# kurhula/pyABC

Hardware: AMD Instinct MI355X
Metric: accepted particles/sec/generation (higher is better)
Workload: dtype f32 (f16x3-limb MFMA, f32-grade)

## Files before the change

### pyabc_amd/csrc/abc_mvn_x3.hip

```cpp
#include "abc_common.h"

namespace abc {
namespace {

typedef _Float16 half8 __attribute__((ext_vector_type(8)));
typedef float f32x16 __attribute__((ext_vector_type(16)));

constexpr double LOG2E = 1.4426950408889634074;
constexpr double SQRT_LOG2E = 1.2011224087864498;
constexpr double LN2 = 0.69314718055994530942;
constexpr int MAX_R = 25;
constexpr int E_MIN = 3, E_MAX = 8;
constexpr float O_MIN = -64.f;
constexpr size_t HDR = 256;
constexpr int X3_PAD = 8;
constexpr int TR = 32;

struct Header { double maxsq; int E; int ok; };

__host__ __device__ constexpr int x3_g0(int r) { return (r + 7 + 7) / 8; }
__host__ __device__ constexpr int x3_k0pad(int r) { return 8 * x3_g0(r); }
__host__ __device__ constexpr int x3_kb(int r) { return (x3_k0pad(r) + 5 * r + 4 + 15) / 16; }
__host__ __device__ constexpr int x3_kb0(int r) { return (x3_g0(r) + 1) / 2; }
static_assert(x3_kb(10) == 5, "K = 80 at r = 10");

struct Limbs3 { double a1, a2, a3; };
struct Limbs5 { double c[5]; };

__device__ __forceinline__ Limbs3 split_coord(double v, int E) {
  Limbs3 L;
  const double G = ldexp(1.0, E - 11);
  L.a1 = rint(v / G);
  double r = v - L.a1 * G;
  L.a2 = rint(ldexp(r / G, 11));
  r -= ldexp(L.a2 * G, -11);
  L.a3 = rint(ldexp(r / G, 22));
  return L;
}

__device__ __forceinline__ int scalar_exp(int l, int E) { return 2 * E - 22 + 22 - 11 * l; }

__device__ __forceinline__ Limbs5 split_scalar(double c, int E) {
  Limbs5 L;
  double r = c;
  for (int l = 0; l < 5; ++l) {
    const int e = scalar_exp(l, E);
    L.c[l] = rint(ldexp(r, -e));
    r -= ldexp(L.c[l], e);
  }
  return L;
}

__device__ __forceinline__ float opv(double limb, int e) { return (float)ldexp(limb, e); }

template <int SIDE>
__device__ __forceinline__ float slot_value(int k, int r, int K0pad, int E,
                                            const Limbs3* L, const Limbs5& S) {
  if (k < K0pad) {
    const int e0 = 2 * (E - 11);
    if (k < r) {
      const int x = e0 >> 1;
      return opv(L[k].a1, SIDE == 0 ? x : e0 - x);
    }
    const int q = k - r;
    if (q < 6) {
      const int l = q % 3;
      const int e = scalar_exp(l, E);
      const int x = e > 4 ? 4 : e;
      const bool limb_side = (q < 3) == (SIDE == 0);
      return limb_side ? opv(S.c[l], x) : opv(1.0, e - x);
    }
    if (q == 6) return SIDE == 0 ? 1.f : 0.f;
    return 0.f;
  }
  const int q = k - K0pad;
  if (q < 5 * r) {
    const int cls = q / r, dim = q % r;
    const int pa[5] = {1, 2, 1, 2, 3}, pb[5] = {2, 1, 3, 2, 1};
    const int p = SIDE == 0 ? pa[cls] : pb[cls];
    const int etot = 2 * (E - 11) - 11 * (pa[cls] + pb[cls] - 2);
    const int x = etot >> 1;
    const double limb = p == 1 ? L[dim].a1 : (p == 2 ? L[dim].a2 : L[dim].a3);
    return opv(limb, SIDE == 0 ? x : etot - x);
  }
  const int e4 = q - 5 * r;
  if (e4 < 4) {
    const int l = 3 + (e4 & 1);
    const int e = scalar_exp(l, E);
    const int x = e < -24 ? -24 : e;
    const bool limb_side = (e4 < 2) == (SIDE == 0);
    return limb_side ? opv(S.c[l], x) : opv(1.0, e - x);
  }
  return 0.f;
}

template <int RR = MAX_R>
__device__ __forceinline__ double whiten(const double* __restrict__ P, int64_t row,
                                         int d, const double* __restrict__ mu,
                                         const double* __restrict__ U, int r,
                                         double* v) {
  double acc[RR];
#pragma unroll
  for (int k = 0; k < RR; ++k) acc[k] = 0.0;
  for (int q = 0; q < d; ++q) {
    const double xq = P[row * d + q] - mu[q];
#pragma unroll
    for (int k = 0; k < RR; ++k)
      if (k < r) acc[k] += xq * U[q * r + k];
  }
  double h = 0.0;
#pragma unroll
  for (int k = 0; k < RR; ++k) {
    if (k < r) {
      const double a = acc[k] * SQRT_LOG2E;
      v[k] = a;
      h += a * a;
    }
  }
  return 0.5 * h;
}

constexpr int POP_RANGE_BLOCKS = 1024;
__global__ __launch_bounds__(256) void pop_range_kernel(
    const double* __restrict__ X, const double* __restrict__ w, int64_t N,
    int d, const double* __restrict__ mu, const double* __restrict__ U, int r,
    Header* __restrict__ hdr) {
  __shared__ double wm[4];
  double h = 0.0;
  for (int64_t row = (int64_t)blockIdx.x * blockDim.x + threadIdx.x; row < N;
       row += (int64_t)gridDim.x * blockDim.x) {
    if (w[row] > 0.0) {
      double v[MAX_R];
      h = fmax(h, whiten(X, row, d, mu, U, r, v));
    }
  }
  h = wave_max(h);
  if ((threadIdx.x & 63) == 0) wm[threadIdx.x >> 6] = h;
  __syncthreads();
  if (threadIdx.x == 0) {
    h = fmax(fmax(wm[0], wm[1]), fmax(wm[2], wm[3]));
    if (h > 0.0)
      atomicMax((unsigned long long*)&hdr->maxsq,
                (unsigned long long)__double_as_longlong(h));
  }
}

__global__ void x3_setup_kernel(Header* __restrict__ hdr, int r,
                                double* __restrict__ range) {
  const double ymax = sqrt(2.0 * hdr->maxsq);
  int E = (int)ceil(log2(1.25 * ymax + 2.0 * sqrt((double)r) + 4.0));
  if (E < E_MIN) E = E_MIN;
  hdr->E = E;
  hdr->ok = E <= E_MAX ? 1 : 0;
  if (range) { range[0] = ymax; range[1] = (double)E; }
}

template <int SIDE, int R>
__global__ __launch_bounds__(128) void pack_x3_kernel(
    const double* __restrict__ P, const double* __restrict__ w, int64_t n,
    int d, const double* __restrict__ mu, const double* __restrict__ U, int r_rt,
    double log_w_shift, int K0pad_rt, int KB_rt, const Header* __restrict__ hdr,
    _Float16* __restrict__ img, int64_t ntiles, int32_t* __restrict__ flags,
    double* __restrict__ Y, double* __restrict__ lw, int64_t Np,
    const int64_t* __restrict__ hint, float* __restrict__ cand_o, int koff,
    const double* __restrict__ shift_dev, const unsigned int* __restrict__ count_dev) {
  if (count_dev) { const int64_t c = (int64_t)*count_dev; n = c < n ? c : n; }
  constexpr int RR = R > 0 ? R : MAX_R;
  const int r = R > 0 ? R : r_rt;
  const int K0pad = R > 0 ? x3_k0pad(R) : K0pad_rt;
  const int KB = R > 0 ? x3_kb(R) : KB_rt;
  constexpr int NG = R > 0 ? x3_kb(R) * 2 : 0;
  const int64_t row = (int64_t)blockIdx.x * blockDim.x + threadIdx.x;
  if (row >= ntiles * TR) return;
  if (count_dev && (row / TR) * TR >= n) return;
  const int E = hdr->E;
  const bool ok = hdr->ok != 0;
  const double L2 = ldexp(1.0, 2 * E);
  double v[RR];
  Limbs3 L[RR];
  double scalar = SIDE == 0 ? -L2 : 0.0;
  bool bad = false;
  float hint_o = O_MIN;
  #pragma unroll
  for (int k = 0; k < RR; ++k) v[k] = 0.0;
  if (row < n) {
    const double h = whiten<RR>(P, row, d, mu, U, r, v);
    if (SIDE == 0) {
      const double wj = w[row];
      bad = !(wj > 0.0) || !(2.0 * h <= L2);
      const double sh = shift_dev ? *shift_dev : log_w_shift;
      const double lwj = wj > 0.0 ? (log(wj) + sh) * LOG2E : -INFINITY;
      scalar = bad ? -L2 : fmax(lwj - h, -L2);
#pragma unroll
      for (int k = 0; k < RR; ++k)
        if (k < r) Y[row * r + k] = v[k];
      lw[row] = lwj;
    } else {
      bad = !ok || !(2.0 * h <= L2);
      scalar = bad ? -L2 : -h;
      if (hint && !bad) {
        const int64_t j = hint[row];
        if (j < 0 || j >= Np || !(lw[j] > -INFINITY)) {
          bad = true;
        } else {
          double q = 0.0;
#pragma unroll
          for (int k = 0; k < RR; ++k)
            if (k < r) { const double t = v[k] - Y[j * r + k]; q += t * t; }
          hint_o = (float)fmax(ceil(lw[j] - 0.5 * q), (double)O_MIN);
        }
        scalar = bad ? -L2 : -h;
      }
    }
    if (bad)
      #pragma unroll
  for (int k = 0; k < RR; ++k) v[k] = 0.0;
  }
  if (flags && row < n) flags[row] = bad ? 1 : 0;
  if (cand_o) cand_o[row] = hint_o;
#pragma unroll
  for (int k = 0; k < RR; ++k) L[k] = split_coord(v[k], E);
  const Limbs5 S = split_scalar(scalar, E);
  const int64_t t = row / TR;
  const int rl = (int)(row % TR);
  const int Ktot = 16 * KB;
#pragma unroll
  for (int g = 0; g < (R > 0 ? NG : 1 << 30); ++g) {
    if (g >= Ktot / 8) break;
    half8 frag;
#pragma unroll
    for (int j = 0; j < 8; ++j) {
      const int k = g * 8 + j;
      float val = slot_value<SIDE>(k, r, K0pad, E, L, S);
      if (SIDE == 1 && hint && k == koff) val = -hint_o;
      frag[j] = (_Float16)val;
    }
    const int kb = g >> 1, lane = rl + 32 * (g & 1);
    *reinterpret_cast<half8*>(img + (((t * KB + kb) * 64) + lane) * 8) = frag;
  }
}

__device__ __forceinline__ float max3(float a, float b, float c) {
  return __builtin_elementwise_maximum(__builtin_elementwise_maximum(a, b), c);
}

__device__ __forceinline__ f32x16 mfma32(const half8& a, const half8& b, const f32x16& c) {
  return __builtin_amdgcn_mfma_f32_32x32x16_f16(a, b, c, 0, 0, 0);
}

template <int KB, int CT, bool PASS1>
__device__ __forceinline__ void x3_wave(
    const half8* __restrict__ A, const half8* __restrict__ Bi, int64_t MT,
    int64_t NT, int chunk, int64_t tiles_per_chunk, int64_t ct0, int koff, int kb0,
    double* __restrict__ part_o, double* __restrict__ part_l, int64_t Mpad) {
  const int lane = threadIdx.x & 63;
  const bool off_lane = (lane >> 5) == ((koff >> 3) & 1);
  const int off_kb = koff >> 4, off_j = koff & 7;

  half8 b[CT][KB];
#pragma unroll
  for (int c = 0; c < CT; ++c) {
    const int64_t ct = ct0 + c < MT ? ct0 + c : MT - 1;
#pragma unroll
    for (int kb = 0; kb < KB; ++kb) b[c][kb] = Bi[(ct * KB + kb) * 64 + lane];
  }
  const int64_t t_begin = (int64_t)chunk * tiles_per_chunk;
  const int64_t t_end = t_begin + tiles_per_chunk < NT ? t_begin + tiles_per_chunk : NT;
  const half8* __restrict__ Al = A + lane;
  static_assert(X3_PAD >= 7, "pad must cover the prefetch distance");
  auto tile = [&](int64_t t) { return t * KB; };
  const f32x16 zero16 = {0.f, 0.f, 0.f, 0.f, 0.f, 0.f, 0.f, 0.f,
                         0.f, 0.f, 0.f, 0.f, 0.f, 0.f, 0.f, 0.f};

  float o[CT];
  if (PASS1 && t_begin < t_end) {
    float mx[CT];
#pragma unroll
    for (int c = 0; c < CT; ++c) mx[c] = -INFINITY;
    half8 ring[4][2];
#pragma unroll
    for (int u = 0; u < 4; ++u)
#pragma unroll
      for (int kb = 0; kb < 2; ++kb)
        if (kb < KB) ring[u][kb] = Al[(tile(t_begin + u) + kb) * 64];
    for (int64_t t = t_begin; t < t_end; t += 4) {
#pragma unroll
      for (int u = 0; u < 4; ++u) {
        if (t + u < t_end) {
#pragma unroll
          for (int c = 0; c < CT; ++c) {
            f32x16 acc = mfma32(ring[u][0], b[c][0], zero16);
            if (KB > 1 && kb0 > 1) acc = mfma32(ring[u][1], b[c][1 < KB ? 1 : 0], acc);
            float m = mx[c];
#pragma unroll
            for (int i = 0; i < 16; i += 2) m = max3(m, acc[i], acc[i + 1]);
            mx[c] = m;
          }
        }
#pragma unroll
        for (int kb = 0; kb < 2; ++kb)
          if (kb < KB) ring[u][kb] = Al[(tile(t + u + 4) + kb) * 64];
      }
    }
#pragma unroll
    for (int c = 0; c < CT; ++c) {
      const float cm = fmaxf(mx[c], __shfl_xor(mx[c], 32, 64));
      o[c] = fmaxf(ceilf(cm), O_MIN);
#pragma unroll
      for (int kb = 0; kb < KB; ++kb)
        if (kb == off_kb && off_lane) b[c][kb][off_j] = (_Float16)(-o[c]);
    }
  } else {
#pragma unroll
    for (int c = 0; c < CT; ++c) o[c] = O_MIN;
  }

  double l64[CT];
  float ls[CT];
#pragma unroll
  for (int c = 0; c < CT; ++c) { l64[c] = 0.0; ls[c] = 0.f; }
  half8 a0[KB], a1[KB];
  if (t_begin < t_end) {
#pragma unroll
    for (int kb = 0; kb < KB; ++kb) {
      a0[kb] = Al[(tile(t_begin) + kb) * 64];
      a1[kb] = Al[(tile(t_begin + 1) + kb) * 64];
    }
  }
  auto chain = [&](const half8 (&a)[KB], int c) {
    f32x16 r = mfma32(a[0], b[c][0], zero16);
#pragma unroll
    for (int kb = 1; kb < KB; ++kb) r = mfma32(a[kb], b[c][kb], r);
    return r;
  };
  auto expsum = [&](const f32x16& v) {
    float e[16];
#pragma unroll
    for (int i = 0; i < 16; ++i) e[i] = __builtin_amdgcn_exp2f(v[i]);
#pragma unroll
    for (int w = 8; w >= 1; w >>= 1)
#pragma unroll
      for (int i = 0; i < w; ++i) e[i] += e[i + w];
    return e[0];
  };
  auto do_tile = [&](const half8 (&a)[KB]) {
    f32x16 prev = chain(a, 0);
#pragma unroll
    for (int c = 1; c < CT; ++c) {
      const f32x16 cur = chain(a, c);
      ls[c - 1] += expsum(prev);
      prev = cur;
    }
    ls[CT - 1] += expsum(prev);
  };
  int nflush = 0;
  for (int64_t t = t_begin; t < t_end; t += 2) {
    do_tile(a0);
#pragma unroll
    for (int kb = 0; kb < KB; ++kb) a0[kb] = Al[(tile(t + 2) + kb) * 64];
    if (t + 1 < t_end) {
      do_tile(a1);
#pragma unroll
      for (int kb = 0; kb < KB; ++kb) a1[kb] = Al[(tile(t + 3) + kb) * 64];
    }
    if (++nflush == 2) {
      nflush = 0;
#pragma unroll
      for (int c = 0; c < CT; ++c) { l64[c] += (double)ls[c]; ls[c] = 0.f; }
    }
  }
#pragma unroll
  for (int c = 0; c < CT; ++c) l64[c] += (double)ls[c];
#pragma unroll
  for (int c = 0; c < CT; ++c) {
    double v = l64[c];
    v += __shfl_xor(v, 32, 64);
    const int64_t ct = ct0 + c;
    if (lane < 32 && ct < MT) {
      if (PASS1) part_o[(int64_t)chunk * Mpad + ct * TR + lane] = (double)o[c];
      part_l[(int64_t)chunk * Mpad + ct * TR + lane] = v;
    }
  }
}

template <int KB, int CT, bool PASS1>
__global__ __launch_bounds__(256) void mvn_x3_kernel(
    const half8* __restrict__ A, const half8* __restrict__ Bi, int64_t MT,
    int64_t NT, int nchunk, int64_t tiles_per_chunk, int64_t ngroups, int koff, int kb0,
    double* __restrict__ part_o, double* __restrict__ part_l, int64_t Mpad,
    const unsigned int* __restrict__ count_dev) {
  const int wave = threadIdx.x >> 6;
  const int64_t bid = blockIdx.x;
  const int cpx = nchunk >> 3;
  const int64_t xcd = bid & 7, jb = bid >> 3;
  const int chunk = (int)(xcd + 8 * (jb % cpx));
  const int64_t gstride = (int64_t)gridDim.x / nchunk;
  const int64_t cnt = count_dev ? (int64_t)*count_dev : MT * TR;
  for (int64_t group = jb / cpx; group < ngroups; group += gstride) {
    const int64_t ct0 = (group * 4 + wave) * CT;
    if (ct0 * TR >= cnt) break;
    x3_wave<KB, CT, PASS1>(A, Bi, MT, NT, chunk, tiles_per_chunk, ct0, koff, kb0, part_o,
                           part_l, Mpad);
  }
}

__global__ void x3_combine_kernel(const double* __restrict__ part_o,
                                  const double* __restrict__ part_l, int nchunk,
                                  int64_t M, int64_t Mpad, double log_const,
                                  const int32_t* __restrict__ cflags,
                                  const float* __restrict__ cand_o,
                                  double* __restrict__ out,
                                  int64_t* __restrict__ rescue,
                                  unsigned int* __restrict__ nrescue,
                                  const unsigned int* __restrict__ count_dev) {
  const int64_t i = (int64_t)blockIdx.x * blockDim.x + threadIdx.x;
  if (i >= M || (count_dev && i >= (int64_t)*count_dev)) return;
  double om = -INFINITY;
  double s = 0.0;
  if (cand_o) {
    om = (double)cand_o[i];
    for (int c = 0; c < nchunk; ++c) s += part_l[(int64_t)c * Mpad + i];
  } else {
    for (int c = 0; c < nchunk; ++c)
      if (part_l[(int64_t)c * Mpad + i] > 0.0) om = fmax(om, part_o[(int64_t)c * Mpad + i]);
    for (int c = 0; c < nchunk; ++c) {
      const double l = part_l[(int64_t)c * Mpad + i];
      if (l > 0.0) s += l * exp2(part_o[(int64_t)c * Mpad + i] - om);
    }
  }
  const double lg = om + log2(s);
  if (cflags[i] || !(s > 0.0) || !(lg >= -60.0) || (cand_o && lg - om > 20.0)) {
    const unsigned int q = atomicAdd(nrescue, 1u);
    rescue[q] = i;
    out[i] = -INFINITY;
    return;
  }
  out[i] = log_const + LN2 * lg;
}

__global__ __launch_bounds__(256) void x3_combine_rows_kernel(
    const double* __restrict__ part_o, const double* __restrict__ part_l, int nchunk,
    int64_t M, int64_t Mpad, double log_const, const int32_t* __restrict__ cflags,
    double* __restrict__ out, int64_t* __restrict__ rescue,
    unsigned int* __restrict__ nrescue, const unsigned int* __restrict__ count_dev) {
  const int lane = threadIdx.x & 63;
  const int64_t i = (int64_t)blockIdx.x * 4 + (threadIdx.x >> 6);
  if (i >= M || i >= (int64_t)*count_dev) return;
  double om = -INFINITY;
  for (int c = lane; c < nchunk; c += 64)
    if (part_l[(int64_t)c * Mpad + i] > 0.0) om = fmax(om, part_o[(int64_t)c * Mpad + i]);
  for (int m = 32; m >= 1; m >>= 1) om = fmax(om, __shfl_xor(om, m, 64));
  double s = 0.0;
  for (int c = lane; c < nchunk; c += 64) {
    const double l = part_l[(int64_t)c * Mpad + i];
    if (l > 0.0) s += l * exp2(part_o[(int64_t)c * Mpad + i] - om);
  }
  for (int m = 32; m >= 1; m >>= 1) s += __shfl_xor(s, m, 64);
  if (lane) return;
  const double lg = om + log2(s);
  if (cflags[i] || !(s > 0.0) || !(lg >= -60.0)) {
    const unsigned int q = atomicAdd(nrescue, 1u);
    rescue[q] = i;
    out[i] = -INFINITY;
    return;
  }
  out[i] = log_const + LN2 * lg;
}

__device__ __forceinline__ void online_add(double s, double& m, double& l) {
  const double dl = s - m;
  if (dl > 0.0) { l = l * exp2(-dl) + 1.0; m = s; }
  else l += (double)__builtin_amdgcn_exp2f((float)dl);
}

constexpr int RS_ROWS = 4096;
constexpr int RS_MAXS = 256;
constexpr int RS_GY = 8;

__host__ __device__ inline int rescue_slices(int64_t N) {
  const int64_t s = (N + RS_ROWS - 1) / RS_ROWS;
  return (int)(s < 1 ? 1 : (s > RS_MAXS ? RS_MAXS : s));
}

__global__ __launch_bounds__(64) void x3_rescue_kernel(
    const int64_t* __restrict__ rescue, const unsigned int* __restrict__ nrescue,
    int64_t q0, int64_t cap, const double* __restrict__ x, int d,
    const double* __restrict__ mu, const double* __restrict__ U, int r,
    const double* __restrict__ Y, const double* __restrict__ lw, int64_t N,
    double* __restrict__ pm, double* __restrict__ pl) {
  __shared__ double ty[64 * MAX_R];
  __shared__ double tl[64];
  const int64_t n = (int64_t)*nrescue;
  const int64_t nq = n - q0 < cap ? n - q0 : cap;
  const int lane = threadIdx.x;
  const int ns = gridDim.x;
  const int64_t per = (N + ns - 1) / ns;
  const int64_t j0 = (int64_t)blockIdx.x * per;
  const int64_t j1 = j0 + per < N ? j0 + per : N;
  for (int64_t g0 = (int64_t)blockIdx.y * 64; g0 < nq; g0 += (int64_t)gridDim.y * 64) {
    const int64_t q = g0 + lane;
    const bool act = q < nq;
    double z[MAX_R];
    const int64_t i = act ? rescue[q0 + q] : 0;
#pragma unroll
    for (int k = 0; k < MAX_R; ++k) {
      if (k < r) {
        double acc = 0.0;
        for (int cc = 0; cc < d; ++cc) acc += (x[i * d + cc] - mu[cc]) * U[cc * r + k];
        z[k] = acc * SQRT_LOG2E;
      }
    }
    double m = -INFINITY, l = 0.0;
    for (int64_t jt = j0; jt < j1; jt += 64) {
      const int cnt = (int)(j1 - jt < 64 ? j1 - jt : 64);
      __syncthreads();
      for (int e = lane; e < cnt * r; e += 64) ty[e] = Y[jt * r + e];
      if (lane < cnt) tl[lane] = lw[jt + lane];
      __syncthreads();
      for (int t = 0; t < cnt; ++t) {
        const double lwj = tl[t];
        if (!(lwj > -INFINITY)) continue;
        double q2 = 0.0;
#pragma unroll
        for (int k = 0; k < MAX_R; ++k) {
          if (k < r) {
            const double dz = z[k] - ty[t * r + k];
            q2 = fma(dz, dz, q2);
          }
        }
        online_add(lwj - 0.5 * q2, m, l);
      }
    }
    if (act) {
      pm[(int64_t)blockIdx.x * cap + q] = m;
      pl[(int64_t)blockIdx.x * cap + q] = l;
    }
  }
}

__global__ void x3_rescue_final(const int64_t* __restrict__ rescue,
                                const unsigned int* __restrict__ nrescue, int64_t q0,
                                int64_t cap, int nslice, const double* __restrict__ pm,
                                const double* __restrict__ pl, double log_const,
                                double* __restrict__ out) {
  const int64_t q = (int64_t)blockIdx.x * blockDim.x + threadIdx.x;
  const int64_t n = (int64_t)*nrescue;
  if (q >= cap || q0 + q >= n) return;
  double mx = -INFINITY;
  for (int c = 0; c < nslice; ++c)
    if (pl[(int64_t)c * cap + q] > 0.0) mx = fmax(mx, pm[(int64_t)c * cap + q]);
  double t = 0.0;
  for (int c = 0; c < nslice; ++c) {
    const double l = pl[(int64_t)c * cap + q];
    if (l > 0.0) t += l * exp2(pm[(int64_t)c * cap + q] - mx);
  }
  out[rescue[q0 + q]] = t > 0.0 ? log_const + LN2 * (mx + log2(t)) : -INFINITY;
}

template <int SIDE>
void launch_pack(int r, dim3 grid, hipStream_t s, const double* P, const double* w,
                 int64_t n, int d, const double* mu, const double* U,
                 double log_w_shift, int K0pad, int KB, const Header* hdr,
                 _Float16* img, int64_t ntiles, int32_t* flags, double* Y,
                 double* lw, int64_t Np, const int64_t* hint, float* cand_o,
                 int koff, const double* shift_dev = nullptr,
                 const unsigned int* count_dev = nullptr) {
#define ABC_PACK_CASE(RC)                                                          \
  case RC:                                                                         \
    hipLaunchKernelGGL((pack_x3_kernel<SIDE, RC>), grid, dim3(128), 0, s, P, w, n, \
                       d, mu, U, r, log_w_shift, K0pad, KB, hdr, img, ntiles, flags, \
                       Y, lw, Np, hint, cand_o, koff, shift_dev, count_dev);       \
    break;
  switch (r) {
    ABC_PACK_CASE(1) ABC_PACK_CASE(2) ABC_PACK_CASE(3) ABC_PACK_CASE(4)
    ABC_PACK_CASE(5) ABC_PACK_CASE(6) ABC_PACK_CASE(7) ABC_PACK_CASE(8)
    ABC_PACK_CASE(9) ABC_PACK_CASE(10) ABC_PACK_CASE(12) ABC_PACK_CASE(16)
    default: ABC_PACK_CASE(0)
  }
#undef ABC_PACK_CASE
}

__global__ void x3_gather_rescued(const int64_t* __restrict__ rescue,
                                  const unsigned int* __restrict__ nres, int64_t cap,
                                  const double* __restrict__ x, int d,
                                  double* __restrict__ xs) {
  const int64_t e = (int64_t)blockIdx.x * blockDim.x + threadIdx.x;
  const int64_t n = (int64_t)*nres < cap ? (int64_t)*nres : cap;
  if (e >= n * d) return;
  xs[e] = x[rescue[e / d] * d + e % d];
}
__global__ void x3_scatter_rescued(const int64_t* __restrict__ rescue,
                                   const unsigned int* __restrict__ nres, int64_t cap,
                                   const double* __restrict__ outs,
                                   double* __restrict__ out) {
  const int64_t q = (int64_t)blockIdx.x * blockDim.x + threadIdx.x;
  if (q < (int64_t)*nres && q < cap) out[rescue[q]] = outs[q];
}

__host__ __device__ constexpr int x3_ct(int KB) {
  return KB <= 3 ? 8 : (KB <= 5 ? 6 : (KB == 6 ? 4 : (KB == 7 ? 3 : 2)));
}

struct PlanX3 {
  int K0pad, KB, KB0, CT, nchunk;
  int64_t MT, NT, MTpad, groups, tiles_per_chunk, Mpad;
};

PlanX3 make_plan_x3(int64_t M, int64_t N, int r, bool fine = false) {
  PlanX3 p;
  p.K0pad = x3_k0pad(r);
  p.KB = x3_kb(r);
  p.KB0 = x3_kb0(r);
  p.CT = x3_ct(p.KB);
  p.MT = ceil_div(M > 0 ? M : 1, TR);
  p.NT = ceil_div(N > 0 ? N : 1, TR);
  const int64_t waves = ceil_div(p.MT, p.CT);
  p.groups = ceil_div(waves, 4);
  p.MTpad = p.groups * 4 * p.CT;
  p.Mpad = p.MTpad * TR;
  int64_t nc = fine ? ceil_div(ceil_div(p.NT, 16), 8) * 8 : ceil_div(ceil_div(p.NT, 128), 8) * 8;
  nc = nc < 8 ? 8 : (nc > (fine ? 256 : 32) ? (fine ? 256 : 32) : nc);
  p.nchunk = (int)nc;
  p.tiles_per_chunk = ceil_div(p.NT, p.nchunk);
  return p;
}

size_t plan_x3_ws(const PlanX3& p) {
  size_t off = 0;
  size_only<_Float16>(off, (size_t)p.MTpad * p.KB * 64 * 8);
  size_only<int32_t>(off, (size_t)p.Mpad);
  size_only<float>(off, (size_t)p.Mpad);
  size_only<double>(off, (size_t)p.nchunk * p.Mpad);
  size_only<double>(off, (size_t)p.nchunk * p.Mpad);
  size_only<int64_t>(off, (size_t)p.Mpad);
  size_only<unsigned int>(off, 64);
  return off + 256;
}

template <int KB, int CT>
void launch_x3(const PlanX3& p, const half8* A, const half8* B, int koff,
               double* po, double* pl, bool pass1, const unsigned int* count_dev,
               hipStream_t s) {
  static_assert(CT == x3_ct(KB), "the plan's tiles per wave must match the instantiation");
  const int64_t gg = count_dev && p.groups > 16 ? 16 : p.groups;
  const int64_t blocks = gg * p.nchunk;
  if (pass1)
    hipLaunchKernelGGL((mvn_x3_kernel<KB, CT, true>), dim3((unsigned)blocks),
                       dim3(256), 0, s, A, B, p.MT, p.NT, p.nchunk,
                       p.tiles_per_chunk, p.groups, koff, p.KB0, po, pl, p.Mpad, count_dev);
  else
    hipLaunchKernelGGL((mvn_x3_kernel<KB, CT, false>), dim3((unsigned)blocks),
                       dim3(256), 0, s, A, B, p.MT, p.NT, p.nchunk,
                       p.tiles_per_chunk, p.groups, koff, p.KB0, po, pl, p.Mpad, count_dev);
}

int dispatch_x3(const PlanX3& p, const half8* A, const half8* B, int koff,
                double* po, double* pl, bool pass1, const unsigned int* count_dev,
                hipStream_t s) {
  switch (p.KB) {
#define ABC_X3_CASE(K) \
  case K: launch_x3<K, x3_ct(K)>(p, A, B, koff, po, pl, pass1, count_dev, s); break;
    ABC_X3_CASE(2) ABC_X3_CASE(3) ABC_X3_CASE(4) ABC_X3_CASE(5) ABC_X3_CASE(6)
    ABC_X3_CASE(7) ABC_X3_CASE(8) ABC_X3_CASE(9) ABC_X3_CASE(10) ABC_X3_CASE(11)
#undef ABC_X3_CASE
    default:
      return set_error(ABC_ERR_UNSUPPORTED, "mvn x3: KB=%d unsupported", p.KB);
  }
  return ABC_OK;
}
static_assert(x3_kb(MAX_R) <= 11 && x3_kb(1) >= 2, "dispatch_x3 covers every rank");

}

size_t x3_frag_bytes(int64_t N, int r) {
  const int KB = x3_kb(r);
  const int64_t NT = ceil_div(N > 0 ? N : 1, TR) + X3_PAD;
  return align_up((size_t)NT * KB * 64 * 8 * sizeof(_Float16), 256);
}
double* x3_Y(const void* packed, int64_t N, int r) {
  return (double*)((char*)packed + HDR + x3_frag_bytes(N, r));
}
double* x3_lw(const void* packed, int64_t N, int r) {
  return x3_Y(packed, N, r) + align_up((size_t)(N > 0 ? N : 1) * r, 32);
}
size_t x3_packed_bytes(int64_t N, int r) {
  return HDR + x3_frag_bytes(N, r) +
         sizeof(double) * (align_up((size_t)(N > 0 ? N : 1) * r, 32) + (N > 0 ? N : 1));
}

int x3_max_rank() { return MAX_R; }

extern "C" int abc_mvn_x3_layout(int r, int* kslots, int* tiles_per_wave) {
  const int KB = x3_kb(r);
  if (kslots) *kslots = 16 * KB;
  if (tiles_per_wave) *tiles_per_wave = x3_ct(KB);
  return 1;
}

int x3_pack_population(const double* X, const double* w, int64_t N, int d,
                       const double* mu, const double* U, int r,
                       double log_w_shift, const double* shift_dev, void* packed,
                       double* range, hipStream_t s) {
  if (r > MAX_R)
    return set_error(ABC_ERR_UNSUPPORTED, "mvn x3: rank %d > %d", r, MAX_R);
  const int64_t NT = ceil_div(N > 0 ? N : 1, TR);
  Header* hdr = (Header*)packed;
  ABC_HIP(hipMemsetAsync(hdr, 0, HDR, s));
  if (N > 0) {
    const int64_t nb = ceil_div(N, 256);
    hipLaunchKernelGGL(pop_range_kernel,
                       dim3((unsigned)(nb < POP_RANGE_BLOCKS ? nb : POP_RANGE_BLOCKS)), dim3(256),
                       0, s, X, w, N, d, mu, U, r, hdr);
    ABC_LAUNCHED();
  }
  hipLaunchKernelGGL(x3_setup_kernel, dim3(1), dim3(1), 0, s, hdr, r, range);
  ABC_LAUNCHED();
  launch_pack<0>(r, dim3((unsigned)ceil_div(NT * TR, 128)), s, X, w, N, d, mu, U,
                 log_w_shift, x3_k0pad(r), x3_kb(r), (const Header*)hdr,
                 (_Float16*)((char*)packed + HDR), NT, (int32_t*)nullptr,
                 x3_Y(packed, N, r), x3_lw(packed, N, r), N, (const int64_t*)nullptr,
                 (float*)nullptr, 0, shift_dev);
  ABC_LAUNCHED();
  return ABC_OK;
}

constexpr int64_t X3_NEST_CAP = 16384;
inline int64_t x3_nest_rows(int64_t M) { return M < X3_NEST_CAP ? M : X3_NEST_CAP; }

size_t x3_logpdf_workspace(int64_t M, int64_t N, int r) {
  const size_t main = plan_x3_ws(make_plan_x3(M, N, r));
  const int64_t m1 = x3_nest_rows(M > 0 ? M : 1);
  size_t nested = 0;
  size_only<double>(nested, (size_t)m1 * 64);
  size_only<double>(nested, (size_t)m1);
  size_only<char>(nested, plan_x3_ws(make_plan_x3(m1, N, r, true)));
  return main + nested + 256;
}

static void x3_rescue_fp64(const PlanX3& p, int64_t q_begin, int64_t M, const double* x, int d,
                    const void* packed, int64_t N, const double* mu, const double* U, int r,
                    double log_const, const int64_t* rescue, const unsigned int* nres,
                    double* po, double* pl, double* out, hipStream_t s) {
  const int ns = rescue_slices(N);
  const int64_t cap = (int64_t)p.nchunk * p.Mpad / ns;
  for (int64_t q0 = q_begin; q0 < M; q0 += cap) {
    hipLaunchKernelGGL(x3_rescue_kernel, dim3((unsigned)ns, (unsigned)RS_GY), dim3(64), 0, s,
                       rescue, nres, q0, cap, x, d, mu, U, r,
                       (const double*)x3_Y(packed, N, r),
                       (const double*)x3_lw(packed, N, r), N, po, pl);
    hipLaunchKernelGGL(x3_rescue_final, dim3((unsigned)ceil_div(cap < M ? cap : M, 256)),
                       dim3(256), 0, s, rescue, nres, q0, cap, ns, po, pl, log_const, out);
  }
}

int x3_logpdf(const double* x, int64_t M, int d, const void* packed,
              const double* X, const double* w, int64_t N, const double* mu,
              const double* U, int r, double log_const, double log_norm,
              double* out, const int64_t* hint, void* ws, size_t ws_bytes,
              hipStream_t s, int prof_channel, const unsigned int* count_dev) {
  if (r > MAX_R)
    return set_error(ABC_ERR_UNSUPPORTED, "mvn x3: rank %d > %d", r, MAX_R);
  PlanX3 p = make_plan_x3(M, N, r, count_dev != nullptr);
  if (ws_bytes < plan_x3_ws(p))
    return set_error(ABC_ERR_WORKSPACE, "mvn x3: workspace %zu < %zu", ws_bytes,
                     plan_x3_ws(p));
  Carver cv(ws, ws_bytes);
  _Float16* Bimg = cv.take<_Float16>((size_t)p.MTpad * p.KB * 64 * 8);
  int32_t* cflags = cv.take<int32_t>((size_t)p.Mpad);
  float* cand_o = cv.take<float>((size_t)p.Mpad);
  double* po = cv.take<double>((size_t)p.nchunk * p.Mpad);
  double* pl = cv.take<double>((size_t)p.nchunk * p.Mpad);
  int64_t* rescue = cv.take<int64_t>((size_t)p.Mpad);
  unsigned int* nres = cv.take<unsigned int>(64);
  if (!cv.ok) return set_error(ABC_ERR_WORKSPACE, "mvn x3: workspace carve");
  const Header* hdr = (const Header*)packed;
  const half8* Aimg = (const half8*)((const char*)packed + HDR);
  ABC_HIP(hipMemsetAsync(nres, 0, sizeof(unsigned int), s));
  launch_pack<1>(r, dim3((unsigned)ceil_div(p.MTpad * TR, 128)), s, x,
                 (const double*)nullptr, M, d, mu, U, log_norm - log_const, p.K0pad,
                 p.KB, hdr, Bimg, p.MTpad, cflags, x3_Y(packed, N, r),
                 x3_lw(packed, N, r), N, hint, hint ? cand_o : (float*)nullptr, r + 6,
                 (const double*)nullptr, count_dev);
  ABC_LAUNCHED();
  profile_start(s, prof_channel);
  int rc = dispatch_x3(p, Aimg, (const half8*)Bimg, r + 6, po, pl, hint == nullptr,
                       count_dev, s);
  profile_stop(s, prof_channel);
  if (rc) return rc;
  ABC_LAUNCHED();
  if (count_dev && !hint)
    hipLaunchKernelGGL(x3_combine_rows_kernel, dim3((unsigned)ceil_div(M, 4)), dim3(256),
                       0, s, po, pl, p.nchunk, M, p.Mpad, log_const, cflags, out, rescue,
                       nres, count_dev);
  else
    hipLaunchKernelGGL(x3_combine_kernel, dim3((unsigned)ceil_div(M, 256)), dim3(256),
                       0, s, po, pl, p.nchunk, M, p.Mpad, log_const, cflags,
                       hint ? (const float*)cand_o : (const float*)nullptr, out,
                       rescue, nres, count_dev);
  ABC_LAUNCHED();
  if (hint) {
    const int64_t Mn = x3_nest_rows(M);
    Carver sub(cv.rest(), cv.rest_bytes());
    double* xs = sub.take<double>((size_t)Mn * d);
    double* outs = sub.take<double>((size_t)Mn);
    const size_t need = plan_x3_ws(make_plan_x3(Mn, N, r, true));
    void* ws2 = sub.take<char>(need);
    if (!sub.ok) return set_error(ABC_ERR_WORKSPACE, "mvn x3: nested rescue workspace");
    hipLaunchKernelGGL(x3_gather_rescued, dim3((unsigned)ceil_div(Mn * d, 256)),
                       dim3(256), 0, s, rescue, nres, Mn, x, d, xs);
    ABC_LAUNCHED();
    const int rc2 = x3_logpdf(xs, Mn, d, packed, X, w, N, mu, U, r, log_const, log_norm,
                              outs, nullptr, ws2, need, s, ABC_PROF_RESCUE, nres);
    if (rc2) return rc2;
    hipLaunchKernelGGL(x3_scatter_rescued, dim3((unsigned)ceil_div(Mn, 256)), dim3(256), 0,
                       s, rescue, nres, Mn, outs, out);
    ABC_LAUNCHED();
    if (M > Mn) {
      x3_rescue_fp64(p, Mn, M, x, d, packed, N, mu, U, r, log_const, rescue, nres, po, pl,
                     out, s);
      ABC_LAUNCHED();
    }
    return ABC_OK;
  }
  x3_rescue_fp64(p, 0, M, x, d, packed, N, mu, U, r, log_const, rescue, nres, po, pl, out, s);
  ABC_LAUNCHED();
  return ABC_OK;
}

}
```

Before: 6.945 million.

## Software-pipeline exp2 reduction into MFMA chain gaps with pinned scheduling

Restructures the inner tile loop so each unit's MFMA chain interleaves the exp2 and tree-sum of the previous unit's accumulator at fixed gaps, using sched_barrier pins to force the ordering. Tile loads move to a helper that keeps offsets in scalar registers with lane byte offsets, and ct0 is made wave-uniform through readfirstlane. The goal is to hide transcendental and add latency behind matrix-core work and to cut VGPR address arithmetic. In exchange, the hand-fixed schedule may block better compiler scheduling, and the tail and flush logic for odd tile counts becomes more complex.

New measurement: 7.386 million (median of 6 runs). 1.06x the previous value.

```diff
diff --git a/pyabc_amd/csrc/abc_mvn_x3.hip b/pyabc_amd/csrc/abc_mvn_x3.hip
--- a/pyabc_amd/csrc/abc_mvn_x3.hip
+++ b/pyabc_amd/csrc/abc_mvn_x3.hip
@@ -248,12 +248,103 @@
   return __builtin_amdgcn_mfma_f32_32x32x16_f16(a, b, c, 0, 0, 0);
 }
 
+template <int KB>
+__device__ __forceinline__ void ld_tile(half8 (&a)[KB], const half8* __restrict__ image,
+                                        int64_t frag, uint32_t& lane_bytes) {
+  static_assert(sizeof(half8) * 64 == 1024, "fragment bytes");
+#pragma unroll
+  for (int g = 0; g < (KB + 3) / 4; ++g) {
+    int64_t off = frag * 1024 + g * 4096;
+    asm volatile("" : "+s"(off));
+#pragma unroll
+    for (int kb = 4 * g; kb < KB && kb < 4 * g + 4; ++kb) {
+      asm volatile("" : "+v"(lane_bytes));
+      a[kb] = *reinterpret_cast<const half8*>(reinterpret_cast<const char*>(image) + off +
+                                              lane_bytes + (kb - 4 * g) * 1024);
+    }
+  }
+}
+
+struct X3Tail { float e3, e11, e7, e15, b1, c0; };
+
+#define X3_PIN() __builtin_amdgcn_sched_barrier(0)
+
+__device__ __forceinline__ void x3_tail_ops(const X3Tail& tl, float& ls) {
+  const float a3 = tl.e3 + tl.e11; X3_PIN();
+  const float a7 = tl.e7 + tl.e15; X3_PIN();
+  const float b3 = a3 + a7; X3_PIN();
+  const float c1 = tl.b1 + b3; X3_PIN();
+  const float dd = tl.c0 + c1; X3_PIN();
+  ls += dd; X3_PIN();
+}
+
+template <int KB>
+__device__ __forceinline__ f32x16 x3_unit(const half8 (&a)[KB], const half8 (&b)[KB],
+                                          const f32x16& v, X3Tail& tl, float& ls_tl) {
+  static_assert(KB >= 2, "gap 0 carries the tail, the exp2 need a later gap");
+  const f32x16 zero16 = {0.f, 0.f, 0.f, 0.f, 0.f, 0.f, 0.f, 0.f,
+                         0.f, 0.f, 0.f, 0.f, 0.f, 0.f, 0.f, 0.f};
+  auto gap = [](int q) { return 1 + q * (KB - 1) / 4; };
+#define X3_E(i) const float e##i = __builtin_amdgcn_exp2f(v[i]); X3_PIN()
+#define X3_A(r, x, y) const float r = x + y; X3_PIN()
+  f32x16 acc = mfma32(a[0], b[0], zero16);
+  X3_PIN();
+  x3_tail_ops(tl, ls_tl);
+  float a0_ = 0.f, a2_ = 0.f, a1_ = 0.f, b0_ = 0.f, e4_ = 0.f, e12_ = 0.f, e6_ = 0.f,
+        e14_ = 0.f, e5_ = 0.f, e13_ = 0.f;
+#pragma unroll
+  for (int kb = 1; kb < KB; ++kb) {
+    acc = mfma32(a[kb], b[kb], acc);
+    X3_PIN();
+    if (gap(0) == kb) {
+      X3_E(0); X3_E(8); X3_E(4); X3_E(12);
+      X3_A(a0, e0, e8);
+      a0_ = a0; e4_ = e4; e12_ = e12;
+    }
+    if (gap(1) == kb) {
+      X3_E(2);
+      X3_A(a4, e4_, e12_);
+      X3_E(10);
+      X3_A(b0, a0_, a4);
+      X3_E(6); X3_E(14);
+      X3_A(a2, e2, e10);
+      b0_ = b0; a2_ = a2; e6_ = e6; e14_ = e14;
+    }
+    if (gap(2) == kb) {
+      X3_E(1);
+      X3_A(a6, e6_, e14_);
+      X3_E(9);
+      X3_A(b2, a2_, a6);
+      X3_E(5);
+      X3_A(c0, b0_, b2);
+      X3_E(13);
+      X3_A(a1, e1, e9);
+      tl.c0 = c0; a1_ = a1; e5_ = e5; e13_ = e13;
+    }
+    if (gap(3) == kb) {
+      X3_E(3);
+      X3_A(a5, e5_, e13_);
+      X3_E(11);
+      X3_A(b1, a1_, a5);
+      X3_E(7); X3_E(15);
+      tl.e3 = e3; tl.e11 = e11; tl.e7 = e7; tl.e15 = e15; tl.b1 = b1;
+    }
+  }
+#undef X3_E
+#undef X3_A
+  return acc;
+}
+
 template <int KB, int CT, bool PASS1>
 __device__ __forceinline__ void x3_wave(
     const half8* __restrict__ A, const half8* __restrict__ Bi, int64_t MT,
-    int64_t NT, int chunk, int64_t tiles_per_chunk, int64_t ct0, int koff, int kb0,
+    int64_t NT, int chunk, int64_t tiles_per_chunk, int64_t ct0_lanes, int koff, int kb0,
     double* __restrict__ part_o, double* __restrict__ part_l, int64_t Mpad) {
   const int lane = threadIdx.x & 63;
+  uint32_t lane_bytes = (uint32_t)lane * (uint32_t)sizeof(half8);
+  const int64_t ct0 =
+      (int64_t)(((uint64_t)(uint32_t)__builtin_amdgcn_readfirstlane((int)(ct0_lanes >> 32)) << 32) |
+                (uint32_t)__builtin_amdgcn_readfirstlane((int)ct0_lanes));
   const bool off_lane = (lane >> 5) == ((koff >> 3) & 1);
   const int off_kb = koff >> 4, off_j = koff & 7;
 
@@ -261,8 +352,7 @@
 #pragma unroll
   for (int c = 0; c < CT; ++c) {
     const int64_t ct = ct0 + c < MT ? ct0 + c : MT - 1;
-#pragma unroll
-    for (int kb = 0; kb < KB; ++kb) b[c][kb] = Bi[(ct * KB + kb) * 64 + lane];
+    ld_tile<KB>(b[c], Bi, ct * KB, lane_bytes);
   }
   const int64_t t_begin = (int64_t)chunk * tiles_per_chunk;
   const int64_t t_end = t_begin + tiles_per_chunk < NT ? t_begin + tiles_per_chunk : NT;
@@ -319,58 +409,67 @@
   float ls[CT];
 #pragma unroll
   for (int c = 0; c < CT; ++c) { l64[c] = 0.0; ls[c] = 0.f; }
-  half8 a0[KB], a1[KB];
+  static_assert(CT >= 2, "a tile's units 0 and 1 are placed apart");
   if (t_begin < t_end) {
-#pragma unroll
-    for (int kb = 0; kb < KB; ++kb) {
-      a0[kb] = Al[(tile(t_begin) + kb) * 64];
-      a1[kb] = Al[(tile(t_begin + 1) + kb) * 64];
-    }
-  }
-  auto chain = [&](const half8 (&a)[KB], int c) {
-    f32x16 r = mfma32(a[0], b[c][0], zero16);
-#pragma unroll
-    for (int kb = 1; kb < KB; ++kb) r = mfma32(a[kb], b[c][kb], r);
-    return r;
-  };
-  auto expsum = [&](const f32x16& v) {
-    float e[16];
-#pragma unroll
-    for (int i = 0; i < 16; ++i) e[i] = __builtin_amdgcn_exp2f(v[i]);
-#pragma unroll
-    for (int w = 8; w >= 1; w >>= 1)
-#pragma unroll
-      for (int i = 0; i < w; ++i) e[i] += e[i + w];
-    return e[0];
-  };
-  auto do_tile = [&](const half8 (&a)[KB]) {
-    f32x16 prev = chain(a, 0);
-#pragma unroll
-    for (int c = 1; c < CT; ++c) {
-      const f32x16 cur = chain(a, c);
-      ls[c - 1] += expsum(prev);
-      prev = cur;
-    }
-    ls[CT - 1] += expsum(prev);
-  };
-  int nflush = 0;
-  for (int64_t t = t_begin; t < t_end; t += 2) {
-    do_tile(a0);
-#pragma unroll
-    for (int kb = 0; kb < KB; ++kb) a0[kb] = Al[(tile(t + 2) + kb) * 64];
-    if (t + 1 < t_end) {
-      do_tile(a1);
-#pragma unroll
-      for (int kb = 0; kb < KB; ++kb) a1[kb] = Al[(tile(t + 3) + kb) * 64];
-    }
-    if (++nflush == 2) {
-      nflush = 0;
+    half8 a0[KB], a1[KB];
+    ld_tile<KB>(a0, A, tile(t_begin), lane_bytes);
+    X3_PIN();
+    ld_tile<KB>(a1, A, tile(t_begin + 1), lane_bytes);
+    X3_PIN();
+    auto expsum = [&](const f32x16& v) {
+      float e[16];
+#pragma unroll
+      for (int i = 0; i < 16; ++i) e[i] = __builtin_amdgcn_exp2f(v[i]);
+#pragma unroll
+      for (int w = 8; w >= 1; w >>= 1)
+#pragma unroll
+        for (int i = 0; i < w; ++i) e[i] += e[i + w];
+      return e[0];
+    };
+    auto flush = [&]() {
 #pragma unroll
       for (int c = 0; c < CT; ++c) { l64[c] += (double)ls[c]; ls[c] = 0.f; }
-    }
-  }
-#pragma unroll
-  for (int c = 0; c < CT; ++c) l64[c] += (double)ls[c];
+    };
+    X3Tail tail = {0.f, 0.f, 0.f, 0.f, 0.f, 0.f};
+    f32x16 prev = mfma32(a0[0], b[0][0], zero16);
+#pragma unroll
+    for (int kb = 1; kb < KB; ++kb) prev = mfma32(a0[kb], b[0][kb], prev);
+    auto rest_of_tile = [&](const half8 (&a)[KB], bool group_start) {
+      prev = x3_unit<KB>(a, b[1], prev, tail, ls[CT - 1]);
+      if (group_start) flush();
+#pragma unroll
+      for (int c = 2; c < CT; ++c) prev = x3_unit<KB>(a, b[c], prev, tail, ls[c - 2]);
+    };
+    auto tile_pair = [&](int64_t t, bool group_start) {
+      rest_of_tile(a0, group_start);
+      ld_tile<KB>(a0, A, tile(t + 2), lane_bytes);
+      X3_PIN();
+      prev = x3_unit<KB>(a1, b[0], prev, tail, ls[CT - 2]);
+      rest_of_tile(a1, false);
+      ld_tile<KB>(a1, A, tile(t + 3), lane_bytes);
+      X3_PIN();
+      prev = x3_unit<KB>(a0, b[0], prev, tail, ls[CT - 2]);
+    };
+    const int64_t nt = t_end - t_begin;
+    int64_t t = t_begin;
+    for (int64_t g = nt >> 2; g > 0; --g, t += 4) {
+      tile_pair(t, true);
+      tile_pair(t + 2, false);
+    }
+    if (nt & 2) {
+      tile_pair(t, true);
+      t += 2;
+    }
+    if (nt & 1) {
+      rest_of_tile(a0, (nt & 2) == 0);
+      x3_tail_ops(tail, ls[CT - 2]);
+      ls[CT - 1] += expsum(prev);
+    } else {
+      x3_tail_ops(tail, ls[CT - 1]);
+    }
+#pragma unroll
+    for (int c = 0; c < CT; ++c) l64[c] += (double)ls[c];
+  }
 #pragma unroll
   for (int c = 0; c < CT; ++c) {
     double v = l64[c];
@@ -382,6 +481,7 @@
     }
   }
 }
+#undef X3_PIN
 
 template <int KB, int CT, bool PASS1>
 __global__ __launch_bounds__(256) void mvn_x3_kernel(
```
